# xiph/daala

Hardware: NVIDIA H100
Metric: encoder Mpixels/s on 4K YUV420 intra (higher is better)
Workload: dtype int32

## Files before the change

daala_b200/csrc/kf_engine.cu:

```cuda
#include <cuda_runtime.h>
#include <math.h>
#include <stdint.h>
#include <stdio.h>
#include <stdlib.h>
#include <string.h>

#include <mutex>

#include "daala_b200.h"
#include "dering_search.h"
#include "gen/coding_order.inc"
#include "pvq_math.cuh"
#include "pvq_warp.cuh"
#include "pvq_common.cuh"

namespace daala_b200 {
namespace kf {

using namespace daala_b200::pvq;

enum Cnt {
  kNLuma = 0, kNChroma, kLumaCoefs, kChromaCoefs,
  kNItemsL = 4,
  kNItemsC = 7,
  kTotalHi = 14,
  kNHeads = 15,
  kNHeads0 = 16,
  kError = 17,
  kHeadLoL = 32,
  kHeadLoC = 64,
  kHeadHi = 96,
  kTailHi = 128,
  kDoneHi = 160,
  kHeadCh = 192,
  kWaiters = 224,
  kCntWords = 256
};

constexpr int kTile = 1024;
constexpr int kMaxLevels = 4096;
constexpr int kLevelBins = kMaxLevels * 3;

struct Lists {
  const uint8_t* bsize;
  int bstride;
  long long bsize_pitch;
  int F, UW, UH;
  int u_row0, u_rows;
  int ntiles;
  int4* tile_sum;
  int32_t* unit_lbase;
  daala_b200_pvq_block* luma;
  daala_b200_pvq_block* chroma;
  int32_t* dep_top;
  int32_t* dep_left;
  int32_t* succ_bottom;
  int32_t* succ_right;
  uint32_t* items_l[3];
  uint32_t* items_c[3];
  uint32_t* heads;
  uint32_t* heads0;
  int32_t* cnt;
  int32_t* lvl_hist;
  int32_t* lvl_cursor;
  uint32_t* lvl_items;
  int nlevels;
  int max_luma, max_chroma;
};

__device__ __forceinline__ int4 add4(int4 a, int4 b) { return make_int4(a.x + b.x, a.y + b.y, a.z + b.z, a.w + b.w); }

__device__ __forceinline__ int4 unit_counts(int b, int ux, int uy) {
  if (b == 0) return make_int4(4, 64, 1, 16);
  const int span = 1 << (b - 1);
  if ((ux & (span - 1)) | (uy & (span - 1))) return make_int4(0, 0, 0, 0);
  const int lc = b == 1 ? 64 : b == 2 ? 256 : 512;
  const int cc = b == 1 ? 16 : b == 2 ? 64 : b == 3 ? 256 : 512;
  return make_int4(1, lc, 1, cc);
}

__device__ __forceinline__ bool unit_of(const Lists& L, long long i, int* f, int* uy, int* ux, int* b) {
  const long long per = (long long)L.u_rows * L.UW;
  if (i >= per * L.F) return false;
  *f = (int)(i / per);
  const int r = (int)(i - (long long)*f * per);
  *uy = L.u_row0 + r / L.UW;
  *ux = r % L.UW;
  *b = L.bsize[*f * L.bsize_pitch + (long long)*uy * L.bstride + *ux];
  return true;
}

__global__ void __launch_bounds__(kTile) k_unit_tile_sums(const __grid_constant__ Lists L) {
  __shared__ int4 part[32];
  const long long i = (long long)blockIdx.x * kTile + threadIdx.x;
// ... 22 lines not shown
  const int t = threadIdx.x;
  if (t == 0) carry = make_int4(0, 0, 0, 0);
  __syncthreads();
  for (int base = 0; base < L.ntiles; base += 1024) {
    const int i = base + t;
    const int4 v = i < L.ntiles ? L.tile_sum[i] : make_int4(0, 0, 0, 0);
    part[t] = v;
    __syncthreads();
    for (int o = 1; o < 1024; o <<= 1) {
      const int4 a = t >= o ? part[t - o] : make_int4(0, 0, 0, 0);
      __syncthreads();
      part[t] = add4(part[t], a);
      __syncthreads();
    }
    const int4 incl = part[t], c = carry;
    if (i < L.ntiles) L.tile_sum[i] = make_int4(c.x + incl.x - v.x, c.y + incl.y - v.y, c.z + incl.z - v.z, c.w + incl.w - v.w);
    __syncthreads();
    if (t == 1023) carry = add4(c, incl);
    __syncthreads();
  }
  if (t == 0) {
    const int4 tot = carry;
    L.cnt[kNLuma] = tot.x;
    L.cnt[kLumaCoefs] = tot.y;
    L.cnt[kNChroma] = 2 * tot.z;
    L.cnt[kChromaCoefs] = 2 * tot.w;
    for (int c = 0; c < 3; c++) {
      L.cnt[kNItemsL + c] = 0;
      L.cnt[kNItemsC + c] = 0;
    }
    L.cnt[kTotalHi] = 0;
    L.cnt[kNHeads] = 0;
    L.cnt[kNHeads0] = 0;
    L.cnt[kError] = tot.x > L.max_luma || 2 * tot.z > L.max_chroma ? 1 : 0;
  }
}

__device__ __forceinline__ void put_block(daala_b200_pvq_block* dst, int coef_off, int x0, int y0, int bs, int pli,
                                          int xdec, int frame) {
  int32_t* w = reinterpret_cast<int32_t*>(dst);
  w[0] = coef_off;
  w[1] = (x0 & 0xffff) | (y0 << 16);
  w[2] = bs | (pli << 8) | (xdec << 16) | (frame << 24);
}

__global__ void __launch_bounds__(kTile) k_unit_emit(const __grid_constant__ Lists L) {
  __shared__ int4 wsum[32];
  const long long i = (long long)blockIdx.x * kTile + threadIdx.x;
  const int lane = threadIdx.x & 31, warp = threadIdx.x >> 5;
  int f = 0, uy = 0, ux = 0, b = 0;
  const bool valid = unit_of(L, i, &f, &uy, &ux, &b);
  const int4 v = valid ? unit_counts(b, ux, uy) : make_int4(0, 0, 0, 0);
  int4 s = v;
#pragma unroll
  for (int o = 1; o < 32; o <<= 1) {
    int4 a;
    a.x = __shfl_up_sync(0xffffffffu, s.x, o);
    a.y = __shfl_up_sync(0xffffffffu, s.y, o);
    a.z = __shfl_up_sync(0xffffffffu, s.z, o);
    a.w = __shfl_up_sync(0xffffffffu, s.w, o);
    if (lane >= o) s = add4(s, a);
  }
  if (lane == 31) wsum[warp] = s;
  __syncthreads();
  int4 pre = L.tile_sum[blockIdx.x];
  for (int w = 0; w < warp; w++) pre = add4(pre, wsum[w]);
  pre = make_int4(pre.x + s.x - v.x, pre.y + s.y - v.y, pre.z + s.z - v.z, pre.w + s.w - v.w);
  if (!valid) return;
  L.unit_lbase[((long long)f * L.UH + uy) * L.UW + ux] = pre.x;
  if (v.x == 0) return;
  if (pre.x + v.x > L.max_luma || 2 * (pre.z + v.z) > L.max_chroma) return;
  if (b == 0) {
    for (int q = 0; q < 4; q++)
      put_block(L.luma + pre.x + q, pre.y + 16 * q, ux * 8 + (q & 1) * 4, uy * 8 + (q >> 1) * 4, 0, 0, 0, f);
  } else {
    put_block(L.luma + pre.x, pre.y, ux * 8, uy * 8, b, 0, 0, f);
  }
  const int cbs = (b > 1 ? b : 1) - 1;
  const int xd = 1 | (b == 0 ? 0x80 : 0);
  put_block(L.chroma + 2 * pre.z, 2 * pre.w, ux * 4, uy * 4, cbs, 1, xd, f);
  put_block(L.chroma + 2 * pre.z + 1, 2 * pre.w + v.w, ux * 4, uy * 4, cbs, 2, xd, f);
}

__device__ __forceinline__ int band_class(int band) { return band < 3 ? 0 : band < 6 ? 1 : 2; }

__device__ __forceinline__ int level_bin(int band, int bs, int x0, int y0, int y_first) {
  const int sh = bs + 2, bx = x0 >> sh, by = (y0 - y_first) >> sh;
  const int r = band % 3;
  const int lvl = band == 0 ? bx + by : r == 1 ? by : bx;
  return lvl * 3 + (2 - band_class(band));
}

__device__ __forceinline__ void append(uint32_t* list, int32_t* counter, bool pred, uint32_t v) {
  const unsigned m = __ballot_sync(__activemask(), pred);
  if (!pred) return;
  const int lane = threadIdx.x & 31, leader = __ffs(m) - 1;
  int base = 0;
  if (lane == leader) base = atomicAdd(counter, __popc(m));
  base = __shfl_sync(m, base, leader);
  list[base + __popc(m & ((1u << lane) - 1u))] = v;
}

__global__ void __launch_bounds__(256) k_luma_deps(const __grid_constant__ Lists L) {
  const int n = min(L.cnt[kNLuma], L.max_luma);
  const int nth = gridDim.x * blockDim.x;
  for (int base = blockIdx.x * blockDim.x; base < n; base += nth) {
    const int blk = base + threadIdx.x;
    const bool in = blk < n;
    int bs = 0, top = -1, left = -1;
    if (in) {
      const daala_b200_pvq_block b = L.luma[blk];
      const int x0 = b.x0, y0 = b.y0, f = b.frame;
      bs = b.bs;
      const int nn = 4 << bs;
      const uint8_t* map = L.bsize + f * L.bsize_pitch;
      if (y0 - nn >= L.u_row0 * 8 && map[(long long)((y0 - 1) >> 3) * L.bstride + (x0 >> 3)] == bs) {
        const int ty = y0 - nn;
        top = L.unit_lbase[((long long)f * L.UH + (ty >> 3)) * L.UW + (x0 >> 3)] +
              (bs == 0 ? ((ty >> 2) & 1) * 2 + ((x0 >> 2) & 1) : 0);
      }
      if (x0 > 0 && map[(long long)(y0 >> 3) * L.bstride + ((x0 - 1) >> 3)] == bs) {
        const int lx = x0 - nn;
        left = L.unit_lbase[((long long)f * L.UH + (y0 >> 3)) * L.UW + (lx >> 3)] +
               (bs == 0 ? ((y0 >> 2) & 1) * 2 + ((lx >> 2) & 1) : 0);
      }
      L.dep_top[blk] = top;
      L.dep_left[blk] = left;
      if (top >= 0) L.succ_bottom[top] = blk;
      if (left >= 0) L.succ_right[left] = blk;
    }
    const int nb = in ? num_bands(bs) : 0;
    int chain = 0;
    for (int band = 0; band < 9; band++) {
      const bool has = band < nb;
      const bool is_free = band == 3 || band == 6;
      const int r = band % 3;
      const bool waits = band == 0 ? (top >= 0 || left >= 0) : r == 1 ? top >= 0 : left >= 0;
      const uint32_t item = ((uint32_t)blk << 4) | band;
      if (band == 3 || band == 6) append(L.items_l[band_class(band)], &L.cnt[kNItemsL + band_class(band)], has, item);
      else if (band == 0) append(L.heads0, &L.cnt[kNHeads0], has && !waits, item);
      else append(L.heads, &L.cnt[kNHeads], has && !waits, item);
      chain += has && !is_free;
      if (has && !is_free && L.lvl_hist) {
        const daala_b200_pvq_block b = L.luma[blk];
        atomicAdd(&L.lvl_hist[level_bin(band, bs, b.x0, b.y0, L.u_row0 * 8)], 1);
      }
    }
#pragma unroll
    for (int o = 16; o > 0; o >>= 1) chain += __shfl_xor_sync(0xffffffffu, chain, o);
    if ((threadIdx.x & 31) == 0 && chain) atomicAdd(&L.cnt[kTotalHi], chain);
  }
}

__global__ void __launch_bounds__(1024) k_level_scan(const __grid_constant__ Lists L) {
  __shared__ int part[1024];
  constexpr int kPer = kLevelBins / 1024;
  const int t = threadIdx.x;
  int v[kPer], sum = 0;
#pragma unroll
  for (int i = 0; i < kPer; i++) {
    v[i] = L.lvl_hist[t * kPer + i];
    sum += v[i];
  }
  part[t] = sum;
  __syncthreads();
  for (int o = 1; o < 1024; o <<= 1) {
    const int add = t >= o ? part[t - o] : 0;
    __syncthreads();
    part[t] += add;
    __syncthreads();
  }
  int run = part[t] - sum;
#pragma unroll
  for (int i = 0; i < kPer; i++) {
    L.lvl_hist[t * kPer + i] = run;
    L.lvl_cursor[t * kPer + i] = run;
    run += v[i];
  }
}

__global__ void __launch_bounds__(256) k_level_scatter(const __grid_constant__ Lists L) {
  const int n = min(L.cnt[kNLuma], L.max_luma);
  for (int blk = blockIdx.x * blockDim.x + threadIdx.x; blk < n; blk += gridDim.x * blockDim.x) {
    const daala_b200_pvq_block b = L.luma[blk];
    const int nb = num_bands(b.bs);
    for (int band = 0; band < nb; band++) {
      if (band == 3 || band == 6) continue;
      const int pos = atomicAdd(&L.lvl_cursor[level_bin(band, b.bs, b.x0, b.y0, L.u_row0 * 8)], 1);
      L.lvl_items[pos] = ((uint32_t)blk << 4) | band;
    }
  }
}

__global__ void __launch_bounds__(256) k_chroma_items(const __grid_constant__ Lists L) {
  const int n = min(L.cnt[kNChroma], L.max_chroma);
  for (int blk = blockIdx.x * blockDim.x + threadIdx.x; blk < n; blk += gridDim.x * blockDim.x) {
    const int bs = L.chroma[blk].bs;
    const int nb = num_bands(bs);
    for (int band = 0; band < nb; band++) {
      const int c = band_class(band);
      const unsigned m = __activemask();
      const unsigned same = __match_any_sync(m, c);
      const int leader = __ffs(same) - 1, lane = threadIdx.x & 31;
      int base = 0;
      if (lane == leader) base = atomicAdd(&L.cnt[kNItemsC + c], __popc(same));
      base = __shfl_sync(same, base, leader);
      L.items_c[c][base + __popc(same & ((1u << lane) - 1u))] = ((uint32_t)blk << 4) | band;
    }
  }
}

__global__ void __launch_bounds__(256) k_luma_items(const __grid_constant__ Lists L) {
  const int n = min(L.cnt[kNLuma], L.max_luma);
  const int nth = gridDim.x * blockDim.x;
  for (int base = blockIdx.x * blockDim.x; base < n; base += nth) {
    const int blk = base + threadIdx.x;
    const int nb = blk < n ? num_bands(L.luma[blk].bs) : 0;
    for (int band = 0; band < 9; band++) {
      const int c = band_class(band);
      append(L.items_l[c], &L.cnt[kNItemsL + c], band < nb, ((uint32_t)blk << 4) | band);
    }
  }
}

struct Stage {
  daala_b200_pvq_params prm;
  const uint32_t* items[3];
  const uint32_t* heads;
  const uint32_t* heads0;
  uint32_t* ring;
  const int32_t* dep_top;
  const int32_t* dep_left;
  const int32_t* succ_bottom;
  const int32_t* succ_right;
  int32_t* join0;
  int32_t* cnt;
  int n_items_at, head_lo_at, n_blocks_at;
  int max_blocks;
  int16_t* sp_vec[3];
  int32_t* sp_lanes[3];
  int32_t* sp_uni[3];
  int16_t* sp_snap[3];
  int sp_slots[3];
  int sp_chunks[3];
  const int32_t* lvl_off;
  const uint32_t* lvl_items;
  int nlevels, lvl_slots;
  int16_t* lv_vec; int32_t* lv_lanes; int32_t* lv_uni; int16_t* lv_snap;
  int32_t* lv_bar;
  int32_t* pre_ev;
  int16_t* pre_snap;
  int max_waiters;
  int skip_lo;
  const double* rsqrt_tbl;
  int16_t* res_pack;
  const int32_t* cfl_plane;
  long long cfl_pitch;
  int cfl_stride;
};

enum { kGatherLuma = 0, kGatherChroma = 1, kGatherInter = 2 };
template <int kKind>
__global__ void __launch_bounds__(256) k_gather(const __grid_constant__ Stage S) {
  const daala_b200_pvq_params& prm = S.prm;
  const int n = min(S.cnt[S.n_blocks_at], S.max_blocks);
  const int lane = threadIdx.x & 31;
  const int nwarps = (gridDim.x * blockDim.x) >> 5;
  for (int blk = (blockIdx.x * blockDim.x + threadIdx.x) >> 5; blk < n; blk += nwarps) {
    const daala_b200_pvq_block b = prm.blocks[blk];
    const int ln = b.bs + 2;
    const int len = ln >= 5 ? 512 : 1 << (2 * ln);
    const int stride = prm.plane_stride[b.pli];
    const int32_t* src = prm.coef_plane[b.pli] + b.frame * prm.plane_frame_pitch[b.pli] + (size_t)b.y0 * stride + b.x0;
    int32_t* vin = prm.in + b.coef_off;
    if (kKind == kGatherLuma) {
      for (int i = lane; i < len; i += 32) vin[i] = i == 0 ? src[0] : src[scan_to_raster(i, ln, stride)];
    } else if (kKind == kGatherInter) {
      const int32_t* psrc = prm.pred_plane[b.pli] + b.frame * prm.plane_frame_pitch[b.pli] + (size_t)b.y0 * stride + b.x0;
      int32_t* vref = prm.ref + b.coef_off;
      for (int i = lane; i < len; i += 32) {
        const int at = i == 0 ? 0 : scan_to_raster(i, ln, stride);
        vin[i] = src[at];
        vref[i] = psrc[at];
      }
    } else {
      const int32_t* psrc = S.cfl_plane + b.frame * S.cfl_pitch + (size_t)b.y0 * S.cfl_stride + b.x0;
      int32_t* vref = prm.ref + b.coef_off;
      const int qoff = prm.qm_stride + ((((1 << (2 * b.bs)) - 1) << 4) / 3);
      int32_t xy = 0;
      for (int i = lane; i < len; i += 32) {
        const int32_t vi = i == 0 ? src[0] : src[scan_to_raster(i, ln, stride)];
        const int32_t vr = i == 0 ? psrc[0] : psrc[scan_to_raster(i, ln, S.cfl_stride)];
// ... 323 lines not shown
          band_search<0>(lane, B, g.bn, snap, vs, S.rsqrt_tbl);
          band_ctx_store_search(lane, B, lanes);
        } else {
          band_ctx_load_finish(lane, B, g.bn, vec, vs, lanes, uni);
          int itheta, max_theta, k;
          double skip_term;
          const int gain = band_finish<0>(lane, B, snap, vs, prm.out + g.off, prm.ref + g.off, g.bn, g.q, prm.y + g.off,
                                          &itheta, &max_theta, &k, g.beta, &skip_term, prm.is_keyframe, g.pli,
                                          prm.qm_inv + g.qoff, prm.pvq_norm_lambda);
          if (lane == 0) {
            const size_t r = (size_t)g.blk * 9 + g.band;
            prm.res_skip_term[r] = skip_term;
            short4 pk;
            pk.x = (short)gain; pk.y = (short)itheta; pk.z = (short)max_theta; pk.w = (short)k;
            reinterpret_cast<short4*>(S.res_pack)[r] = pk;
          }
        }
      }
      grid_barrier(S.lv_bar, &bar_target, gridDim.x);
    }
  }
}

template <bool kIntra>
__global__ void __launch_bounds__(kPersistThreads, kPersistCtas) k_pvq_persist(const __grid_constant__ Stage S) {
  __shared__ __align__(16) int16_t snap_all[kPersistThreads / 32][kSnapEntries];
  const int lane = threadIdx.x & 31;
  int16_t* snap = snap_all[threadIdx.x >> 5];
  int done = 0;
  bool waiter = false;
  for (;;) {
    uint32_t item = next_item<kIntra>(S, lane, &done, &waiter);
    if (item == kNoItem) return;
    for (;;) {
      const int band = (int)(item & 15);
      run_item<kIntra>(S, item, lane, snap);
      if (!kIntra || band == 3 || band == 6) break;
      done += band == 0;
      __threadfence();
      __syncwarp();
      uint32_t next = kNoItem;
      if (lane == 0) {
        const int blk = (int)(item >> 4);
        if (band == 0) {
          const int nb[2] = {S.succ_bottom[blk], S.succ_right[blk]};
          for (int i = 0; i < 2; i++) {
            if (nb[i] < 0) continue;
            const int need = (S.dep_top[nb[i]] >= 0) + (S.dep_left[nb[i]] >= 0);
            if (need == 2 && atomicAdd(&S.join0[nb[i]], 1) != 1) continue;
            if (next == kNoItem) {
              next = (uint32_t)nb[i] << 4;
            } else {
              __threadfence();
              push_chain(S, nb[i], 0);
            }
          }
        } else {
          const int nb = band % 3 == 1 ? S.succ_bottom[blk] : S.succ_right[blk];
          if (nb >= 0) next = ((uint32_t)nb << 4) | band;
        }
      }
      next = __shfl_sync(0xffffffffu, next, 0);
      if (next == kNoItem) break;
      __threadfence();
      item = next;
    }
  }
}

__global__ void k_fill_rsqrt(double* tbl) {
  const int i = blockIdx.x * blockDim.x + threadIdx.x;
  if (i < kTableDoubles) pvq_fill_rsqrt_table(tbl, i);
}

__global__ void k_begin_pvq(int32_t* cnt, int luma) {
  if (threadIdx.x == 0 && blockIdx.x == 0) {
    if (luma) {
      cnt[kHeadLoL] = 0;
      cnt[kHeadHi] = 0;
      cnt[kTailHi] = cnt[kNHeads0];
      cnt[kDoneHi] = 0;
      cnt[kHeadCh] = 0;
      cnt[kWaiters] = 0;
    } else {
      cnt[kHeadLoC] = 0;
    }
  }
}

template <bool kInter>
__global__ void __launch_bounds__(256) k_finish_scatter(const __grid_constant__ Stage S) {
  const daala_b200_pvq_params& prm = S.prm;
  const int n = min(S.cnt[S.n_blocks_at], S.max_blocks);
  const int lane = threadIdx.x & 31;
  const int nwarps = (gridDim.x * blockDim.x) >> 5;
  for (int blk = (blockIdx.x * blockDim.x + threadIdx.x) >> 5; blk < n; blk += nwarps) {
    const daala_b200_pvq_block b = prm.blocks[blk];
    const int ln = b.bs + 2, nn = 1 << ln;
    const int len = ln >= 5 ? 512 : 1 << (2 * ln);
    const int stride = prm.plane_stride[b.pli];
    int32_t* dst = prm.coef_plane[b.pli] + b.frame * prm.plane_frame_pitch[b.pli] + (size_t)b.y0 * stride + b.x0;
    const int32_t* src = prm.out + b.coef_off;
    if (lane == 0) {
      const int nb = num_bands(b.bs);
      double sd = 0;
      for (int i = 0; i < nb; i++) sd += prm.res_skip_term[(size_t)blk * 9 + i];
      prm.res_skip_diff[blk] = sd;
      if (!kInter) {
        prm.out[b.coef_off] = prm.in[b.coef_off];
      } else {
        int dc_quant = (prm.q0 * prm.pvq_qm_q4[b.pli][b.bs * (b.bs + 1)]) >> 4;
        if (dc_quant < 1) dc_quant = 1;
        const int32_t r = prm.ref[b.coef_off], diff = prm.in[b.coef_off] - r;
        int qdc = 0;
        if (abs(diff) >= dc_quant * 141 / 256) {
          const int half = ((dc_quant + 1) >> 1) - 1;
// ... 467 lines not shown
  if (kf->cfg.level_chains) {
    KF_CHECK(dalloc(kf, &L.lvl_hist, (size_t)kLevelBins));
    KF_CHECK(dalloc(kf, &L.lvl_cursor, (size_t)kLevelBins));
    KF_CHECK(dalloc(kf, &L.lvl_items, kf->chain_cap));
    L.nlevels = (kf->plane_w[0] + L.u_rows * 8) / 4 + 2;
    if (L.nlevels >= kMaxLevels) return (int)cudaErrorInvalidValue;
    kf->lvl_slots = 2048 * F;
    KF_CHECK(dalloc(kf, &kf->lv_vec, (size_t)kf->lvl_slots * 3 * 128));
    KF_CHECK(dalloc(kf, &kf->lv_lanes, (size_t)kf->lvl_slots * kCtxLaneWords * 16));
    KF_CHECK(dalloc(kf, &kf->lv_uni, (size_t)kf->lvl_slots * kCtxUniWords));
    KF_CHECK(dalloc(kf, &kf->lv_snap, (size_t)kf->lvl_slots * kMaxEvents * 128));
    KF_CHECK(dalloc(kf, &kf->lv_bar, (size_t)32));
    int per_sm = 0;
    KF_CHECK(cudaOccupancyMaxActiveBlocksPerMultiprocessor(&per_sm, k_pvq_levels, 128, 0));
    if (per_sm < 1) return (int)cudaErrorLaunchOutOfResources;
    kf->lvl_grid = per_sm * kf->sms;
  }
  {
    const int want = kf->cfg.persist_ctas_per_sm > 0 ? kf->cfg.persist_ctas_per_sm : kPersistCtas;
    int per_sm[2] = {0, 0};
    KF_CHECK(cudaFuncSetAttribute(k_pvq_persist<true>, cudaFuncAttributePreferredSharedMemoryCarveout,
                                  cudaSharedmemCarveoutMaxShared));
    KF_CHECK(cudaFuncSetAttribute(k_pvq_persist<false>, cudaFuncAttributePreferredSharedMemoryCarveout,
                                  cudaSharedmemCarveoutMaxShared));
    KF_CHECK(cudaOccupancyMaxActiveBlocksPerMultiprocessor(&per_sm[0], k_pvq_persist<true>, kPersistThreads, 0));
    KF_CHECK(cudaOccupancyMaxActiveBlocksPerMultiprocessor(&per_sm[1], k_pvq_persist<false>, kPersistThreads, 0));
    if (per_sm[0] < want || per_sm[1] < want) {
      snprintf(kf->err, sizeof(kf->err), "k_pvq_persist: %d / %d CTAs per SM resident, %d wanted", per_sm[0],
               per_sm[1], want);
      return (int)cudaErrorLaunchOutOfResources;
    }
  }
  KF_CHECK(dalloc(kf, &L.heads, inter ? 0 : kf->chain_cap));
  KF_CHECK(dalloc(kf, &L.heads0, ndep));
  KF_CHECK(dalloc(kf, &L.cnt, (size_t)kCntWords));

  auto setup_stage = [&](Stage& S, bool chroma) -> int {
    memset(&S, 0, sizeof(S));
    daala_b200_pvq_params& p = S.prm;
    const size_t ncoef = chroma ? luma_shard_px / 2 + 1024 : luma_shard_px + 1024;
    const size_t nblk = chroma ? L.max_chroma : L.max_luma;
    p.blocks = chroma ? L.chroma : L.luma;
    KF_CHECK(dalloc(kf, &p.in, ncoef));
    KF_CHECK(dalloc(kf, &p.ref, ncoef));
    KF_CHECK(dalloc(kf, &p.out, ncoef));
    KF_CHECK(dalloc(kf, &p.y, ncoef));
    KF_CHECK(dalloc(kf, &p.y16, ncoef));
    KF_CHECK(dalloc(kf, &p.res_skip_term, nblk * 9));
    KF_CHECK(dalloc(kf, &p.res_skip_diff, nblk));
    KF_CHECK(dalloc(kf, &p.res_flip, nblk));
    KF_CHECK(dalloc(kf, &S.res_pack, nblk * 9 * 4));
    p.res_gain = p.res_theta = p.res_max_theta = p.res_k = nullptr;
    p.res_dc = nullptr;
    if (inter) KF_CHECK(dalloc(kf, &p.res_dc, nblk));
    p.qm = kf->qm;
    p.qm_inv = kf->qm_inv;
    for (int i = 0; i < 3; i++) {
      p.coef_plane[i] = kf->coeffs[i];
      p.pred_plane[i] = kf->pred_coeffs[i];
      p.plane_frame_pitch[i] = (long long)kf->plane_w[i] * kf->plane_h[i];
      p.plane_stride[i] = kf->plane_w[i];
    }
    p.qm_stride = kf->cfg.qm_stride;
    p.q0 = kf->cfg.q0 > 1 ? kf->cfg.q0 : 1;
    p.is_keyframe = inter ? 0 : 1;
    p.use_masking = kf->cfg.use_masking;
// ... 2 lines not shown
    for (int c = 0; c < 3; c++) S.items[c] = chroma ? L.items_c[c] : L.items_l[c];
    S.cnt = L.cnt;
    S.rsqrt_tbl = kf->rsqrt_tbl;
    for (int c = 0; c < 3; c++) {
      S.sp_vec[c] = kf->sp_vec[c];
      S.sp_lanes[c] = kf->sp_lanes[c];
      S.sp_uni[c] = kf->sp_uni[c];
      S.sp_snap[c] = kf->sp_snap[c];
      S.sp_slots[c] = kf->sp_slots[c];
      const size_t cap = chroma ? cap_c[c] : cap_l[c];
      S.sp_chunks[c] = kf->sp_slots[c] > 0 ? (int)((cap + kf->sp_slots[c] - 1) / kf->sp_slots[c]) : 0;
    }
    S.skip_lo = chroma ? 0 : kf->cfg.split_free > 1;
    S.max_waiters = getenv("DAALA_B200_MAX_WAITERS") ? atoi(getenv("DAALA_B200_MAX_WAITERS")) : kf->sms * 8;
    if (!chroma && kf->cfg.noref_prepass) {
      KF_CHECK(dalloc(kf, &S.pre_ev, (ncoef / 8 + 2) * kPreEvWords));
      KF_CHECK(dalloc(kf, &S.pre_snap, 2 * ncoef));
    }
    if (!chroma) {
      S.lvl_off = L.lvl_hist;
      S.lvl_items = L.lvl_items;
      S.nlevels = L.nlevels;
      S.lvl_slots = kf->lvl_slots;
      S.lv_vec = kf->lv_vec;
      S.lv_lanes = kf->lv_lanes;
      S.lv_uni = kf->lv_uni;
      S.lv_snap = kf->lv_snap;
      S.lv_bar = kf->lv_bar;
    }
    S.n_items_at = chroma ? kNItemsC : kNItemsL;
    S.head_lo_at = chroma ? kHeadLoC : kHeadLoL;
    S.n_blocks_at = chroma ? kNChroma : kNLuma;
    S.max_blocks = (int)nblk;
    if (!chroma) {
      S.dep_top = L.dep_top;
      S.dep_left = L.dep_left;
      S.succ_bottom = L.succ_bottom;
      S.succ_right = L.succ_right;
      S.heads = L.heads;
      S.heads0 = L.heads0;
      KF_CHECK(dalloc(kf, &S.ring, inter ? 0 : kf->chain_cap));
      KF_CHECK(dalloc(kf, &S.join0, ndep));
    } else {
      S.cfl_plane = kf->cfl_plane;
      S.cfl_pitch = (long long)kf->plane_w[1] * kf->plane_h[1];
      S.cfl_stride = kf->plane_w[1];
    }
    return 0;
  };
  int rc = setup_stage(kf->luma, false);
  if (rc) return rc;
  rc = setup_stage(kf->chroma, true);
  if (rc) return rc;
  (void)luma_px;
  if (kf->cfg.symbol_stream) {
    Sym& Y = kf->sym;
    memset(&Y, 0, sizeof(Y));
    Y.bsize = kf->bsize;
    Y.bstride = UW;
    Y.bsize_pitch = (long long)UW * UH;
    Y.F = F;
    Y.nhsb = kf->nhsb;
    Y.sb_rows = kf->cfg.sb_rows;
    Y.u_row0 = L.u_row0;
    Y.nsb = kf->nhsb * kf->cfg.sb_rows;
    Y.cap_blocks = L.max_luma + L.max_chroma;
// ... 113 lines not shown
  }
  if (phases & DAALA_B200_KF_FORWARD) {
    int rc = daala_b200_launch_forward(&kf->frame, 3, s);
    if (!rc) rc = daala_b200_launch_forward(&kf->frame_pred, 3, s);
    if (rc) return rc;
  }
  const bool core = (phases & DAALA_B200_KF_SEARCH_ONLY) != 0;
  for (const Stage* S : {&kf->luma, &kf->chroma}) {
    if (!(phases & (S == &kf->luma ? DAALA_B200_KF_PVQ_LUMA : DAALA_B200_KF_PVQ_CHROMA))) continue;
    if (!core) k_gather<kGatherInter><<<wide, 256, 0, s>>>(*S);
    enqueue_split<false>(kf, *S, s);
    if (!core) k_finish_scatter<true><<<wide, 256, 0, s>>>(*S);
  }
  if (phases & DAALA_B200_KF_INVERSE) {
    int rc = daala_b200_launch_inverse(&kf->frame, 3, s);
    if (rc) return rc;
  }
  return (int)cudaGetLastError();
}

static int kf_enqueue_step(daala_b200_kf* kf, int phases) {
  if (kf->cfg.inter) return kf_enqueue_step_inter(kf, phases);
  cudaStream_t s = kf->stream;
  const Lists& L = kf->lists;
  const int wide = kf->sms * 8;
  if (phases & DAALA_B200_KF_LISTS) {
    k_unit_tile_sums<<<L.ntiles, kTile, 0, s>>>(L);
    k_tile_scan<<<1, 1024, 0, s>>>(L);
    k_unit_emit<<<L.ntiles, kTile, 0, s>>>(L);
    const size_t nl = (size_t)L.max_luma * sizeof(int32_t);
    if (cudaMemsetAsync(L.succ_bottom, 0xff, nl, s) != cudaSuccess || cudaMemsetAsync(L.succ_right, 0xff, nl, s) != cudaSuccess)
      return (int)cudaGetLastError();
    if (L.lvl_hist && cudaMemsetAsync(L.lvl_hist, 0, sizeof(int32_t) * kLevelBins, s) != cudaSuccess) return (int)cudaGetLastError();
    k_luma_deps<<<wide, 256, 0, s>>>(L);
    if (L.lvl_hist) {
      k_level_scan<<<1, 1024, 0, s>>>(L);
      k_level_scatter<<<wide, 256, 0, s>>>(L);
    }
    k_chroma_items<<<wide, 256, 0, s>>>(L);
  }
  if (phases & DAALA_B200_KF_FORWARD) {
    int rc = daala_b200_launch_forward(&kf->frame, 3, s);
    if (rc) return rc;
  }
  const int persist = kf->sms * (kf->cfg.persist_ctas_per_sm > 0 ? kf->cfg.persist_ctas_per_sm : kPersistCtas);
  const bool core = (phases & DAALA_B200_KF_SEARCH_ONLY) != 0;
  if (phases & DAALA_B200_KF_PVQ_LUMA) {
    if (cudaMemsetAsync(kf->luma.ring, 0xff, kf->chain_cap * sizeof(uint32_t), s) != cudaSuccess ||
        cudaMemsetAsync(kf->luma.join0, 0, (size_t)kf->luma.max_blocks * sizeof(int32_t), s) != cudaSuccess)
      return (int)cudaGetLastError();
    k_begin_pvq<<<1, 32, 0, s>>>(kf->lists.cnt, 1);
    if (!core) k_gather<kGatherLuma><<<wide, 256, 0, s>>>(kf->luma);
    if (kf->cfg.split_free > 1) enqueue_split<true>(kf, kf->luma, s);
    if (kf->luma.pre_ev) {
      k_pvq_prepass<2><<<kf->sms * 16, 128, 0, s>>>(kf->luma);
      k_pvq_prepass<1><<<kf->sms * 16, 128, 0, s>>>(kf->luma);
    }
    if (kf->cfg.level_chains) {
      if (cudaMemsetAsync(kf->lv_bar, 0, sizeof(int32_t) * 32, s) != cudaSuccess) return (int)cudaGetLastError();
      k_pvq_levels<<<kf->lvl_grid, 128, 0, s>>>(kf->luma);
    } else {
      k_pvq_persist<true><<<persist, kPersistThreads, 0, s>>>(kf->luma);
    }
    if (!core) k_finish_scatter<false><<<wide, 256, 0, s>>>(kf->luma);
  }
  if (phases & DAALA_B200_KF_PVQ_CHROMA) {
// ... 157 lines not shown
  if (kf->exec) cudaGraphExecDestroy(kf->exec);
  if (kf->graph) cudaGraphDestroy(kf->graph);
  for (int p = 0; p < 3; p++) {
    cudaFree(kf->pixels[p]);
    cudaFree(kf->coeffs[p]);
    cudaFree(kf->lapped[p]);
    cudaFree(kf->pixels_out[p]);
    cudaFree(kf->pred_pixels[p]);
    cudaFree(kf->pred_coeffs[p]);
  }
  cudaFree(kf->bsize);
  cudaFree(kf->cfl_plane);
  cudaFree(kf->qm);
  cudaFree(kf->qm_inv);
  cudaFree(kf->rsqrt_tbl);
  for (int c = 0; c < 3; c++) {
    cudaFree(kf->sp_vec[c]);
    cudaFree(kf->sp_lanes[c]);
    cudaFree(kf->sp_uni[c]);
    cudaFree(kf->sp_snap[c]);
  }
  Lists& L = kf->lists;
  cudaFree(L.tile_sum);
  cudaFree(L.unit_lbase);
  cudaFree(L.luma);
  cudaFree(L.chroma);
  cudaFree(L.dep_top);
  cudaFree(L.dep_left);
  for (int c = 0; c < 3; c++) {
    cudaFree(L.items_l[c]);
    cudaFree(L.items_c[c]);
  }
  cudaFree(L.heads);
  cudaFree(L.heads0);
  cudaFree(L.lvl_hist);
  cudaFree(L.lvl_cursor);
  cudaFree(L.lvl_items);
  cudaFree(kf->lv_vec);
  cudaFree(kf->lv_lanes);
  cudaFree(kf->lv_uni);
  cudaFree(kf->lv_snap);
  cudaFree(kf->lv_bar);
  cudaFree(kf->dering_level);
  cudaFree(kf->dering_orig);
  cudaFree(kf->dering_cand);
  cudaFree(kf->dering_dist);
  cudaFree(kf->dering_thr[0]);
  cudaFree(kf->dering_thr[1]);
  cudaFree(kf->dering_dir);
  cudaFree(kf->dering_skip);
  for (int p = 0; p < 3; p++) cudaFree(kf->dering_in[p]);
  cudaFree(kf->dering_filt);
  cudaFree(L.succ_bottom);
  cudaFree(L.succ_right);
  cudaFree(L.cnt);
  Sym& Y = kf->sym;
  cudaFree(Y.unit_rank);
  cudaFree(Y.sb_cnt);
  cudaFree(Y.sb_base);
  cudaFree(Y.order);
  cudaFree(Y.off);
  cudaFree(Y.tile);
  cudaFree(Y.tot);
  cudaFree(Y.index);
  cudaFree(Y.blocks);
  cudaFree(Y.bands);
  cudaFree(Y.pulses);
  for (Stage* S : {&kf->luma, &kf->chroma}) {
    cudaFree(S->prm.in);
    cudaFree(S->prm.ref);
    cudaFree(S->prm.out);
    cudaFree(S->prm.y);
    cudaFree(S->prm.y16);
    cudaFree(S->prm.res_skip_term);
    cudaFree(S->prm.res_skip_diff);
    cudaFree(S->prm.res_flip);
    cudaFree(S->prm.res_dc);
    cudaFree(S->res_pack);
    cudaFree(S->ring);
    cudaFree(S->join0);
    cudaFree(S->pre_ev);
    cudaFree(S->pre_snap);
  }
  if (kf->own_stream) cudaStreamDestroy(kf->stream);
  free(kf);
}

const char* daala_b200_kf_error(const daala_b200_kf* kf) { return kf ? kf->err : g_create_err; }

int daala_b200_kf_launches_per_step(const daala_b200_kf* kf) {
  if (!kf) return 0;
  auto split = [](const Stage& S) { return 3 * (S.sp_chunks[0] + S.sp_chunks[1] + S.sp_chunks[2]); };
  if (kf->cfg.inter) return 5 + 2 + (2 + split(kf->luma)) + (2 + split(kf->chroma)) + 2;
  int n = 5 + (kf->cfg.level_chains ? 2 : 0);
  n += 1;
  n += 3 + 1 + (kf->cfg.split_free > 1 ? split(kf->luma) : 0) + (kf->luma.pre_ev ? 2 : 0);
  n += 4 + (kf->cfg.split_free > 0 ? split(kf->chroma) : 1);
  if (!kf->cfg.dering) n += 2;
  else n += 1 + 1 + 1 + 3;
  if (kf->cfg.dering == 2) n += 5 + 6 + 6 + 1;
  if (kf->cfg.symbol_stream) n += 8;
  return n;
}

int daala_b200_kf_device_buffers(daala_b200_kf* kf, daala_b200_kf_buffers* out) {
  if (!kf || !out) return (int)cudaErrorInvalidValue;
  memset(out, 0, sizeof(*out));
  for (int p = 0; p < 3; p++) {
    out->pixels[p] = kf->pixels[p];
    out->coeffs[p] = kf->coeffs[p];
    out->lapped[p] = kf->lapped[p];
    out->pixels_out[p] = kf->pixels_out[p];
    out->plane_w[p] = kf->plane_w[p];
    out->plane_h[p] = kf->plane_h[p];
  }
  out->bsize = kf->bsize;
  out->counts = kf->lists.cnt;
  out->luma_blocks = kf->lists.luma;
  out->chroma_blocks = kf->lists.chroma;
  out->dep_top = kf->lists.dep_top;
  out->dep_left = kf->lists.dep_left;
  for (int c = 0; c < 3; c++) {
    out->luma_items[c] = kf->lists.items_l[c];
    out->chroma_items[c] = kf->lists.items_c[c];
  }
  out->luma_heads = kf->lists.heads;
  out->luma_heads0 = kf->lists.heads0;
  out->succ_bottom = kf->lists.succ_bottom;
  out->succ_right = kf->lists.succ_right;
  out->luma_res = kf->luma.res_pack;
  out->chroma_res = kf->chroma.res_pack;
  out->luma_y16 = kf->luma.prm.y16;
  out->chroma_y16 = kf->chroma.prm.y16;
  out->luma_skip_diff = kf->luma.prm.res_skip_diff;
  out->chroma_skip_diff = kf->chroma.prm.res_skip_diff;
  out->chroma_flip = kf->chroma.prm.res_flip;
  out->max_luma_blocks = kf->lists.max_luma;
  out->max_chroma_blocks = kf->lists.max_chroma;
  out->stream = kf->stream;
  out->bytes_allocated = (long long)kf->bytes_allocated;
  for (int p = 0; p < 3; p++) {
    out->pred_pixels[p] = kf->pred_pixels[p];
    out->pred_coeffs[p] = kf->pred_coeffs[p];
  }
  return 0;
}

int daala_b200_kf_run_device(daala_b200_kf* kf, int phases, int use_graph) {
  if (!kf) return (int)cudaErrorInvalidValue;
  if (!use_graph || phases != DAALA_B200_KF_ALL) return kf_enqueue_step(kf, phases);
  if (!kf->captured) {
    int rc = kf_enqueue_step(kf, phases);
    if (rc) return rc;
    KF_CHECK(cudaStreamSynchronize(kf->stream));
    KF_CHECK(cudaStreamBeginCapture(kf->stream, cudaStreamCaptureModeThreadLocal));
    rc = kf_enqueue_step(kf, phases);
    cudaError_t e = cudaStreamEndCapture(kf->stream, &kf->graph);
    if (rc) return rc;
    KF_CHECK(e);
    KF_CHECK(cudaGraphInstantiate(&kf->exec, kf->graph, 0));
// ... 203 lines not shown
```

daala_b200/engine.py:

```python
import ctypes

import numpy as np

from . import _native, pvq
from .frame import Geometry

c_int, c_ll, c_void_p = ctypes.c_int, ctypes.c_longlong, ctypes.c_void_p

PH_LISTS, PH_FORWARD, PH_PVQ_LUMA, PH_INVERSE, PH_PVQ_CHROMA = 1, 2, 4, 8, 16
PH_PVQ, PH_ALL, PH_SEARCH_ONLY = 20, 31, 64
CNT = dict(n_luma=0, n_chroma=1, luma_coefs=2, chroma_coefs=3, items_l=4, items_c=7,
           total_hi=14, n_heads=15, n_heads0=16, error=17)


class Config(ctypes.Structure):
    _fields_ = [("pic_w", c_int), ("pic_h", c_int), ("nframes", c_int), ("q0", c_int), ("use_masking", c_int),
                ("qm_stride", c_int), ("pvq_norm_lambda", ctypes.c_double), ("pvq_qm_q4", (ctypes.c_ubyte * 32) * 3),
                ("qm", c_void_p), ("qm_inv", c_void_p), ("sb_row0", c_int), ("sb_rows", c_int),
                ("max_blocks_div", c_int), ("persist_ctas_per_sm", c_int), ("split_free", c_int), ("dering", c_int), ("noref_prepass", c_int), ("level_chains", c_int), ("stream", c_void_p),
                ("coded_quantizer", c_int), ("qm_is_flat", c_int), ("dering_lambda", ctypes.c_double),
                ("symbol_stream", c_int), ("inter", c_int)]


class Totals(ctypes.Structure):
    _fields_ = [("n_luma", c_ll), ("luma_coefs", c_ll), ("n_chroma", c_ll), ("chroma_coefs", c_ll)]


class IO(ctypes.Structure):
    _fields_ = [("pixels", c_void_p * 3), ("bsize", c_void_p), ("dering_level", c_void_p), ("totals", ctypes.POINTER(Totals)),
                ("pixels_out", c_void_p * 3), ("luma_blocks", c_void_p), ("chroma_blocks", c_void_p),
                ("luma_res", c_void_p), ("chroma_res", c_void_p), ("luma_y16", c_void_p), ("chroma_y16", c_void_p),
                ("luma_skip_diff", c_void_p), ("chroma_skip_diff", c_void_p), ("chroma_flip", c_void_p),
                ("counts", c_void_p), ("dering_level_out", c_void_p),
                ("sym_index", c_void_p), ("sym_index_cap", c_ll), ("sym_blocks", c_void_p), ("sym_blocks_cap", c_ll),
                ("sym_bands", c_void_p), ("sym_bands_cap", c_ll), ("sym_pulses", c_void_p), ("sym_pulses_cap", c_ll),
                ("pred_pixels", c_void_p * 3), ("luma_dc", c_void_p), ("chroma_dc", c_void_p)]


class SymBounds(ctypes.Structure):
    _fields_ = [("index", c_ll), ("blocks", c_ll), ("bands", c_ll), ("pulse_bytes", c_ll)]


class Buffers(ctypes.Structure):
    _fields_ = [("pixels", c_void_p * 3), ("coeffs", c_void_p * 3), ("lapped", c_void_p * 3),
                ("pixels_out", c_void_p * 3), ("plane_w", c_int * 3), ("plane_h", c_int * 3), ("bsize", c_void_p),
                ("counts", c_void_p), ("luma_blocks", c_void_p), ("chroma_blocks", c_void_p), ("dep_top", c_void_p),
                ("dep_left", c_void_p), ("succ_bottom", c_void_p), ("succ_right", c_void_p), ("luma_items", c_void_p * 3),
                ("luma_heads", c_void_p), ("luma_heads0", c_void_p), ("chroma_items", c_void_p * 3),
                ("luma_res", c_void_p), ("chroma_res", c_void_p), ("luma_y16", c_void_p), ("chroma_y16", c_void_p),
                ("luma_skip_diff", c_void_p), ("chroma_skip_diff", c_void_p), ("chroma_flip", c_void_p),
                ("max_luma_blocks", c_int), ("max_chroma_blocks", c_int), ("stream", c_void_p),
                ("bytes_allocated", c_ll), ("pred_pixels", c_void_p * 3), ("pred_coeffs", c_void_p * 3)]


def _bind():
    L = _native.lib()
    if getattr(L, "_kf_bound", False):
        return L
    L.daala_b200_kf_create.argtypes = [ctypes.POINTER(Config)]
    L.daala_b200_kf_create.restype = c_void_p
    L.daala_b200_kf_destroy.argtypes = [c_void_p]
    L.daala_b200_kf_destroy.restype = None
    L.daala_b200_kf_error.argtypes = [c_void_p]
    L.daala_b200_kf_error.restype = ctypes.c_char_p
    L.daala_b200_kf_device_buffers.argtypes = [c_void_p, ctypes.POINTER(Buffers)]
    L.daala_b200_kf_launches_per_step.argtypes = [c_void_p]
    L.daala_b200_kf_run_device.argtypes = [c_void_p, c_int, c_int]
    L.daala_b200_kf_time_device.argtypes = [c_void_p, c_int, c_int, c_int, ctypes.POINTER(ctypes.c_float)]
    L.daala_b200_kf_count_blocks.argtypes = [c_void_p, c_int, c_ll, c_int, c_int, c_int, c_int, c_int,
                                             ctypes.POINTER(Totals)]
    for name in ("daala_b200_kf_submit", "daala_b200_kf_encode"):
        getattr(L, name).argtypes = [c_void_p, ctypes.POINTER(IO)]
    L.daala_b200_kf_symbol_bounds.argtypes = [ctypes.POINTER(Totals), c_int, ctypes.POINTER(SymBounds)]
    L.daala_b200_kf_wait.argtypes = [c_void_p]
    L.daala_b200_device_copy.argtypes = [c_void_p, c_void_p, ctypes.c_size_t, c_int]
    L.daala_b200_host_alloc.argtypes = [ctypes.c_size_t]
    L.daala_b200_host_alloc.restype = c_void_p
    L.daala_b200_host_free.argtypes = [c_void_p]
    L.daala_b200_host_free.restype = None
    L._kf_bound = True
    return L


class Pinned:

# ... 275 lines not shown
```

include/daala_b200.h:

```cpp
#ifndef DAALA_B200_H
#define DAALA_B200_H

#include <stddef.h>
#include <stdint.h>

#ifdef __cplusplus
extern "C" {
#endif

typedef int32_t od_coeff;


void od_bin_fdct4(od_coeff y[4], const od_coeff *x, int xstride);
void od_bin_idct4(od_coeff *x, int xstride, const od_coeff y[4]);
void od_bin_fdct8(od_coeff y[8], const od_coeff *x, int xstride);
void od_bin_idct8(od_coeff *x, int xstride, const od_coeff y[8]);
void od_bin_fdct16(od_coeff y[16], const od_coeff *x, int xstride);
void od_bin_idct16(od_coeff *x, int xstride, const od_coeff y[16]);
void od_bin_fdct32(od_coeff y[32], const od_coeff *x, int xstride);
void od_bin_idct32(od_coeff *x, int xstride, const od_coeff y[32]);
void od_bin_fdct64(od_coeff y[64], const od_coeff *x, int xstride);
void od_bin_idct64(od_coeff *x, int xstride, const od_coeff y[64]);

void od_bin_fdct4x4(od_coeff *y, int ystride, const od_coeff *x, int xstride);
// ... 309 lines not shown
  daala_b200_kf_sym_block *sym_blocks;
  long long sym_blocks_cap;
  int16_t *sym_bands;
  long long sym_bands_cap;
  uint8_t *sym_pulses;
  long long sym_pulses_cap;
  const uint8_t *pred_pixels[3];
  int32_t *luma_dc, *chroma_dc;
} daala_b200_kf_io;

typedef struct daala_b200_kf_buffers {
  uint8_t *pixels[3];
  int32_t *coeffs[3];
  int32_t *lapped[3];
  uint8_t *pixels_out[3];
  int plane_w[3], plane_h[3];
  uint8_t *bsize;
  int32_t *counts;
  daala_b200_pvq_block *luma_blocks, *chroma_blocks;
  int32_t *dep_top, *dep_left;
  int32_t *succ_bottom, *succ_right;
  uint32_t *luma_items[3];
  uint32_t *luma_heads;
  uint32_t *luma_heads0;
  uint32_t *chroma_items[3];
  int16_t *luma_res, *chroma_res, *luma_y16, *chroma_y16;
  double *luma_skip_diff, *chroma_skip_diff;
  int32_t *chroma_flip;
  int max_luma_blocks, max_chroma_blocks;
  void *stream;
  long long bytes_allocated;
  uint8_t *pred_pixels[3];
  int32_t *pred_coeffs[3];
} daala_b200_kf_buffers;

#define DAALA_B200_KF_LISTS 1
#define DAALA_B200_KF_FORWARD 2
#define DAALA_B200_KF_PVQ_LUMA 4
#define DAALA_B200_KF_INVERSE 8
#define DAALA_B200_KF_PVQ_CHROMA 16
#define DAALA_B200_KF_PVQ (DAALA_B200_KF_PVQ_LUMA | DAALA_B200_KF_PVQ_CHROMA)
#define DAALA_B200_KF_ALL 31
#define DAALA_B200_KF_SEARCH_ONLY 64

daala_b200_kf *daala_b200_kf_create(const daala_b200_kf_config *cfg);
void daala_b200_kf_destroy(daala_b200_kf *kf);
const char *daala_b200_kf_error(const daala_b200_kf *kf);
int daala_b200_kf_device_buffers(daala_b200_kf *kf, daala_b200_kf_buffers *out);
int daala_b200_kf_launches_per_step(const daala_b200_kf *kf);
int daala_b200_kf_run_device(daala_b200_kf *kf, int phases, int use_graph);
int daala_b200_kf_time_device(daala_b200_kf *kf, int phases, int use_graph, int reps, float *ms);
int daala_b200_kf_count_blocks(const uint8_t *bsize, int nframes, long long frame_pitch, int bstride, int nhsb,
                               int nvsb, int sb_row0, int sb_rows, daala_b200_kf_totals *out);
int daala_b200_kf_symbol_bounds(const daala_b200_kf_totals *t, int nframes, daala_b200_kf_sym_bounds *out);
int daala_b200_kf_submit(daala_b200_kf *kf, const daala_b200_kf_io *io);
int daala_b200_kf_wait(daala_b200_kf *kf);
int daala_b200_kf_encode(daala_b200_kf *kf, const daala_b200_kf_io *io);
int daala_b200_device_copy(void *dst, const void *src, size_t bytes, int kind);
void *daala_b200_host_alloc(size_t bytes);
void daala_b200_host_free(void *p);


typedef struct daala_b200_mc_block {
  int32_t mvx[4];
  int32_t mvy[4];
  uint16_t x0, y0;
// ... 38 lines not shown
```

Baseline: 2158.

## Order luma dependency-chain heads by estimated chain length, longest first

Computes, for each chain head, how long its vertical or horizontal dependency chain is. Weighting that length by band class gives a bin, and the heads are sorted by bin with a histogram, a scan run in the last block to finish, and a scatter, so the persistent PVQ workers pick up the longest chains first. The aim is to shorten the critical-path tail of the wavefront schedule. The cost is extra map walks, atomics and buffers in the list-building kernels. It also adds an optional compile-time tracing path that records per-item timing.

```diff
diff --git a/daala_b200/csrc/kf_engine.cu b/daala_b200/csrc/kf_engine.cu
--- a/daala_b200/csrc/kf_engine.cu
+++ b/daala_b200/csrc/kf_engine.cu
@@ -27,6 +27,7 @@
   kNHeads = 15,
   kNHeads0 = 16,
   kError = 17,
+  kDepsDone = 18,
   kHeadLoL = 32,
   kHeadLoC = 64,
   kHeadHi = 96,
@@ -34,6 +35,7 @@
   kDoneHi = 160,
   kHeadCh = 192,
   kWaiters = 224,
+  kTraceN = 240,
   kCntWords = 256
 };
 
@@ -60,6 +62,10 @@
   uint32_t* items_c[3];
   uint32_t* heads;
   uint32_t* heads0;
+  uint32_t* heads_raw;
+  int32_t* head_bin;
+  int32_t* head_hist;
+  int32_t* head_cursor;
   int32_t* cnt;
   int32_t* lvl_hist;
   int32_t* lvl_cursor;
@@ -148,6 +154,7 @@
     L.cnt[kTotalHi] = 0;
     L.cnt[kNHeads] = 0;
     L.cnt[kNHeads0] = 0;
+    L.cnt[kDepsDone] = 0;
     L.cnt[kError] = tot.x > L.max_luma || 2 * tot.z > L.max_chroma ? 1 : 0;
   }
 }
@@ -207,14 +214,71 @@
   return lvl * 3 + (2 - band_class(band));
 }
 
-__device__ __forceinline__ void append(uint32_t* list, int32_t* counter, bool pred, uint32_t v) {
+__device__ __forceinline__ int append(uint32_t* list, int32_t* counter, bool pred, uint32_t v) {
   const unsigned m = __ballot_sync(__activemask(), pred);
-  if (!pred) return;
+  if (!pred) return -1;
   const int lane = threadIdx.x & 31, leader = __ffs(m) - 1;
   int base = 0;
   if (lane == leader) base = atomicAdd(counter, __popc(m));
   base = __shfl_sync(m, base, leader);
-  list[base + __popc(m & ((1u << lane) - 1u))] = v;
+  const int pos = base + __popc(m & ((1u << lane) - 1u));
+  list[pos] = v;
+  return pos;
+}
+
+__device__ __forceinline__ int count_key(int32_t* ctr, int key) {
+  const unsigned same = __match_any_sync(__activemask(), key);
+  const int lane = threadIdx.x & 31, leader = __ffs(same) - 1;
+  int base = 0;
+  if (lane == leader) base = atomicAdd(&ctr[key], __popc(same));
+  return __shfl_sync(same, base, leader) + __popc(same & ((1u << lane) - 1u));
+}
+
+constexpr int kChainCost0 = 7, kChainCost1 = 9, kChainCost2 = 18;
+__device__ __forceinline__ int weight_bin(int len, int band) {
+  const int c = band_class(band);
+  const int w = len * (c == 0 ? kChainCost0 : c == 1 ? kChainCost1 : kChainCost2);
+  return kLevelBins - 1 - min(w, kLevelBins - 1);
+}
+
+__device__ int chain_length(const Lists& L, const uint8_t* map, int x0, int y0, int bs, bool down) {
+  const int nn = 4 << bs, y_end = (L.u_row0 + L.u_rows) * 8, x_end = L.UW * 8;
+  int len = 1;
+  for (int x = x0 + (down ? 0 : nn), y = y0 + (down ? nn : 0); x < x_end && y < y_end;
+       x += down ? 0 : nn, y += down ? nn : 0, len++) {
+    if (map[(long long)(y >> 3) * L.bstride + (x >> 3)] != bs) break;
+    const int py = down ? y - 1 : y, px = down ? x : x - 1;
+    if (map[(long long)(py >> 3) * L.bstride + (px >> 3)] != bs) break;
+  }
+  return len;
+}
+
+template <int kThreads>
+__device__ __forceinline__ void scan_bins(int32_t* hist, int32_t* cursor) {
+  __shared__ int part[kThreads];
+  constexpr int kPer = kLevelBins / kThreads;
+  const int t = threadIdx.x;
+  int v[kPer], sum = 0;
+#pragma unroll
+  for (int i = 0; i < kPer; i++) {
+    v[i] = __ldcg(hist + t * kPer + i);
+    sum += v[i];
+  }
+  part[t] = sum;
+  __syncthreads();
+  for (int o = 1; o < kThreads; o <<= 1) {
+    const int add = t >= o ? part[t - o] : 0;
+    __syncthreads();
+    part[t] += add;
+    __syncthreads();
+  }
+  int run = part[t] - sum;
+#pragma unroll
+  for (int i = 0; i < kPer; i++) {
+    hist[t * kPer + i] = run;
+    cursor[t * kPer + i] = run;
+    run += v[i];
+  }
 }
 
 __global__ void __launch_bounds__(256) k_luma_deps(const __grid_constant__ Lists L) {
@@ -246,6 +310,13 @@
       if (left >= 0) L.succ_right[left] = blk;
     }
     const int nb = in ? num_bands(bs) : 0;
+    int len_down = 0, len_across = 0;
+    if (nb > 1) {
+      const daala_b200_pvq_block b = L.luma[blk];
+      const uint8_t* map = L.bsize + b.frame * L.bsize_pitch;
+      if (top < 0) len_down = chain_length(L, map, b.x0, b.y0, bs, true);
+      if (left < 0) len_across = chain_length(L, map, b.x0, b.y0, bs, false);
+    }
     int chain = 0;
     for (int band = 0; band < 9; band++) {
       const bool has = band < nb;
@@ -253,9 +324,18 @@
       const int r = band % 3;
       const bool waits = band == 0 ? (top >= 0 || left >= 0) : r == 1 ? top >= 0 : left >= 0;
       const uint32_t item = ((uint32_t)blk << 4) | band;
-      if (band == 3 || band == 6) append(L.items_l[band_class(band)], &L.cnt[kNItemsL + band_class(band)], has, item);
-      else if (band == 0) append(L.heads0, &L.cnt[kNHeads0], has && !waits, item);
-      else append(L.heads, &L.cnt[kNHeads], has && !waits, item);
+      if (band == 3 || band == 6) {
+        append(L.items_l[band_class(band)], &L.cnt[kNItemsL + band_class(band)], has, item);
+      } else if (band == 0) {
+        append(L.heads0, &L.cnt[kNHeads0], has && !waits, item);
+      } else {
+        const int pos = append(L.heads_raw, &L.cnt[kNHeads], has && !waits, item);
+        if (pos >= 0) {
+          const int bin = weight_bin(r == 1 ? len_down : len_across, band);
+          L.head_bin[pos] = bin;
+          count_key(L.head_hist, bin);
+        }
+      }
       chain += has && !is_free;
       if (has && !is_free && L.lvl_hist) {
         const daala_b200_pvq_block b = L.luma[blk];
@@ -266,33 +346,19 @@
     for (int o = 16; o > 0; o >>= 1) chain += __shfl_xor_sync(0xffffffffu, chain, o);
     if ((threadIdx.x & 31) == 0 && chain) atomicAdd(&L.cnt[kTotalHi], chain);
   }
+  __shared__ bool last;
+  __threadfence();
+  __syncthreads();
+  if (threadIdx.x == 0) last = atomicAdd(&L.cnt[kDepsDone], 1) == (int)gridDim.x - 1;
+  __syncthreads();
+  if (last) {
+    __threadfence();
+    scan_bins<256>(L.head_hist, L.head_cursor);
+  }
 }
 
 __global__ void __launch_bounds__(1024) k_level_scan(const __grid_constant__ Lists L) {
-  __shared__ int part[1024];
-  constexpr int kPer = kLevelBins / 1024;
-  const int t = threadIdx.x;
-  int v[kPer], sum = 0;
-#pragma unroll
-  for (int i = 0; i < kPer; i++) {
-    v[i] = L.lvl_hist[t * kPer + i];
-    sum += v[i];
-  }
-  part[t] = sum;
-  __syncthreads();
-  for (int o = 1; o < 1024; o <<= 1) {
-    const int add = t >= o ? part[t - o] : 0;
-    __syncthreads();
-    part[t] += add;
-    __syncthreads();
-  }
-  int run = part[t] - sum;
-#pragma unroll
-  for (int i = 0; i < kPer; i++) {
-    L.lvl_hist[t * kPer + i] = run;
-    L.lvl_cursor[t * kPer + i] = run;
-    run += v[i];
-  }
+  scan_bins<1024>(L.lvl_hist, L.lvl_cursor);
 }
 
 __global__ void __launch_bounds__(256) k_level_scatter(const __grid_constant__ Lists L) {
@@ -309,6 +375,9 @@
 }
 
 __global__ void __launch_bounds__(256) k_chroma_items(const __grid_constant__ Lists L) {
+  const int nh = L.cnt[kNHeads];
+  for (int i = blockIdx.x * blockDim.x + threadIdx.x; i < nh; i += gridDim.x * blockDim.x)
+    L.heads[count_key(L.head_cursor, L.head_bin[i])] = L.heads_raw[i];
   const int n = min(L.cnt[kNChroma], L.max_chroma);
   for (int blk = blockIdx.x * blockDim.x + threadIdx.x; blk < n; blk += gridDim.x * blockDim.x) {
     const int bs = L.chroma[blk].bs;
@@ -373,7 +442,49 @@
   const int32_t* cfl_plane;
   long long cfl_pitch;
   int cfl_stride;
+#ifdef DAALA_B200_CHAIN_TRACE
+  struct ChainTraceRec* trace;
+  int trace_cap;
+#endif
 };
+
+#ifdef DAALA_B200_CHAIN_TRACE
+struct ChainTraceRec {
+  unsigned long long t0, t1;
+  uint32_t item;
+  uint32_t cta;
+  uint16_t sm;
+  uint8_t bs;
+  uint8_t kind;
+  uint32_t pad;
+};
+
+__device__ __forceinline__ unsigned long long globaltimer() {
+  unsigned long long t;
+  asm volatile("mov.u64 %0, %%globaltimer;" : "=l"(t));
+  return t;
+}
+
+__device__ __noinline__ void trace_item(const Stage& S, uint32_t item, int kind, unsigned long long t0, int lane) {
+  __syncwarp();
+  if (lane != 0) return;
+  const unsigned long long t1 = globaltimer();
+  const int i = atomicAdd(&S.cnt[kTraceN], 1);
+  if (i >= S.trace_cap) return;
+  uint32_t sm;
+  asm volatile("mov.u32 %0, %%smid;" : "=r"(sm));
+  ChainTraceRec r;
+  r.t0 = t0;
+  r.t1 = t1;
+  r.item = item;
+  r.cta = blockIdx.x;
+  r.sm = (uint16_t)sm;
+  r.bs = (uint8_t)S.prm.blocks[item >> 4].bs;
+  r.kind = (uint8_t)kind;
+  r.pad = 0;
+  S.trace[i] = r;
+}
+#endif
 
 enum { kGatherLuma = 0, kGatherChroma = 1, kGatherInter = 2 };
 template <int kKind>
@@ -763,9 +874,19 @@
   for (;;) {
     uint32_t item = next_item<kIntra>(S, lane, &done, &waiter);
     if (item == kNoItem) return;
+#ifdef DAALA_B200_CHAIN_TRACE
+    int kind = (item & 15) == 0 ? 0 : (item & 15) == 3 || (item & 15) == 6 ? 2 : 1;
+#endif
     for (;;) {
       const int band = (int)(item & 15);
+#ifdef DAALA_B200_CHAIN_TRACE
+      const unsigned long long t0 = globaltimer();
+#endif
       run_item<kIntra>(S, item, lane, snap);
+#ifdef DAALA_B200_CHAIN_TRACE
+      if (kIntra) trace_item(S, item, kind, t0, lane);
+      kind = 3;
+#endif
       if (!kIntra || band == 3 || band == 6) break;
       done += band == 0;
       __threadfence();
@@ -813,6 +934,9 @@
       cnt[kDoneHi] = 0;
       cnt[kHeadCh] = 0;
       cnt[kWaiters] = 0;
+#ifdef DAALA_B200_CHAIN_TRACE
+      cnt[kTraceN] = 0;
+#endif
     } else {
       cnt[kHeadLoC] = 0;
     }
@@ -1346,6 +1470,10 @@
     }
   }
   KF_CHECK(dalloc(kf, &L.heads, inter ? 0 : kf->chain_cap));
+  KF_CHECK(dalloc(kf, &L.heads_raw, inter ? 0 : kf->chain_cap));
+  KF_CHECK(dalloc(kf, &L.head_bin, inter ? 0 : kf->chain_cap));
+  KF_CHECK(dalloc(kf, &L.head_hist, inter ? 0 : (size_t)kLevelBins));
+  KF_CHECK(dalloc(kf, &L.head_cursor, inter ? 0 : (size_t)kLevelBins));
   KF_CHECK(dalloc(kf, &L.heads0, ndep));
   KF_CHECK(dalloc(kf, &L.cnt, (size_t)kCntWords));
 
@@ -1414,6 +1542,12 @@
     S.head_lo_at = chroma ? kHeadLoC : kHeadLoL;
     S.n_blocks_at = chroma ? kNChroma : kNLuma;
     S.max_blocks = (int)nblk;
+#ifdef DAALA_B200_CHAIN_TRACE
+    if (!chroma && !inter) {
+      S.trace_cap = (int)(luma_shard_px / 16);
+      KF_CHECK(dalloc(kf, &S.trace, (size_t)S.trace_cap));
+    }
+#endif
     if (!chroma) {
       S.dep_top = L.dep_top;
       S.dep_left = L.dep_left;
@@ -1593,6 +1727,7 @@
     if (cudaMemsetAsync(L.succ_bottom, 0xff, nl, s) != cudaSuccess || cudaMemsetAsync(L.succ_right, 0xff, nl, s) != cudaSuccess)
       return (int)cudaGetLastError();
     if (L.lvl_hist && cudaMemsetAsync(L.lvl_hist, 0, sizeof(int32_t) * kLevelBins, s) != cudaSuccess) return (int)cudaGetLastError();
+    if (cudaMemsetAsync(L.head_hist, 0, sizeof(int32_t) * kLevelBins, s) != cudaSuccess) return (int)cudaGetLastError();
     k_luma_deps<<<wide, 256, 0, s>>>(L);
     if (L.lvl_hist) {
       k_level_scan<<<1, 1024, 0, s>>>(L);
@@ -1816,6 +1951,10 @@
     cudaFree(L.items_c[c]);
   }
   cudaFree(L.heads);
+  cudaFree(L.heads_raw);
+  cudaFree(L.head_bin);
+  cudaFree(L.head_hist);
+  cudaFree(L.head_cursor);
   cudaFree(L.heads0);
   cudaFree(L.lvl_hist);
   cudaFree(L.lvl_cursor);
@@ -1865,12 +2004,24 @@
     cudaFree(S->join0);
     cudaFree(S->pre_ev);
     cudaFree(S->pre_snap);
+#ifdef DAALA_B200_CHAIN_TRACE
+    cudaFree(S->trace);
+#endif
   }
   if (kf->own_stream) cudaStreamDestroy(kf->stream);
   free(kf);
 }
 
 const char* daala_b200_kf_error(const daala_b200_kf* kf) { return kf ? kf->err : g_create_err; }
+
+#ifdef DAALA_B200_CHAIN_TRACE
+int daala_b200_kf_chain_trace(daala_b200_kf* kf, void** recs, int* cap) {
+  if (!kf || !recs || !cap) return (int)cudaErrorInvalidValue;
+  *recs = kf->luma.trace;
+  *cap = kf->luma.trace_cap;
+  return 0;
+}
+#endif
 
 int daala_b200_kf_launches_per_step(const daala_b200_kf* kf) {
   if (!kf) return 0;
@@ -1910,6 +2061,8 @@
   }
   out->luma_heads = kf->lists.heads;
   out->luma_heads0 = kf->lists.heads0;
+  out->luma_heads_raw = kf->lists.heads_raw;
+  out->luma_head_bin = kf->lists.head_bin;
   out->succ_bottom = kf->lists.succ_bottom;
   out->succ_right = kf->lists.succ_right;
   out->luma_res = kf->luma.res_pack;
diff --git a/daala_b200/engine.py b/daala_b200/engine.py
--- a/daala_b200/engine.py
+++ b/daala_b200/engine.py
@@ -50,7 +50,8 @@
                 ("luma_res", c_void_p), ("chroma_res", c_void_p), ("luma_y16", c_void_p), ("chroma_y16", c_void_p),
                 ("luma_skip_diff", c_void_p), ("chroma_skip_diff", c_void_p), ("chroma_flip", c_void_p),
                 ("max_luma_blocks", c_int), ("max_chroma_blocks", c_int), ("stream", c_void_p),
-                ("bytes_allocated", c_ll), ("pred_pixels", c_void_p * 3), ("pred_coeffs", c_void_p * 3)]
+                ("bytes_allocated", c_ll), ("pred_pixels", c_void_p * 3), ("pred_coeffs", c_void_p * 3),
+                ("luma_heads_raw", c_void_p), ("luma_head_bin", c_void_p)]
 
 
 def _bind():
diff --git a/include/daala_b200.h b/include/daala_b200.h
--- a/include/daala_b200.h
+++ b/include/daala_b200.h
@@ -365,6 +365,8 @@
   long long bytes_allocated;
   uint8_t *pred_pixels[3];
   int32_t *pred_coeffs[3];
+  uint32_t *luma_heads_raw;
+  int32_t *luma_head_bin;
 } daala_b200_kf_buffers;
 
 #define DAALA_B200_KF_LISTS 1
```

Measured after the change: 2367, median of 6. +9.7%, better.
